# onesamblack/distributed-torch-horovod-gcp

Measured on NVIDIA H100. Metric: images/sec (whole job, device-timed, max over ranks) ResNet-50 synthetic ImageNet training, higher is better.
Workload: dtype bf16

## Files before the change

### distributed_torch_horovod_gcp_b200/csrc/conv_sm90.cu

```cuda
#include <cuda.h>
#include <cuda_bf16.h>
#include <cuda_runtime.h>
#include <limits.h>
#include <stdint.h>
#include <stdio.h>
#include <stdlib.h>
#include <string.h>

#include "sm90_common.cuh"

namespace {

constexpr int MAX_TAPS = 9;
constexpr int MAX_CLASSES = 4;

struct ConvTap {
  int amap;
  int dw, dh;
  int wcol;
};
struct ConvClass {
  int ntaps;
  int out_map;
  ConvTap taps[MAX_TAPS];
// ... 279 lines not shown
    for (int r = 0; r < R; ++r)
      for (int c = 0; c < S; ++c) {
        ConvTap& t = cl.taps[cl.ntaps++];
        t.amap = 0; t.dh = pad - r; t.dw = pad - c; t.wcol = (r * S + c) * Cin;
      }
    if (make_map4(&maps.out[0], dx, Cin, W, H, N, Cin, (uint64_t)W * Cin, (uint64_t)H * W * Cin, p.sw, p.sh, sn))
      return -1;
    maps.out[1] = maps.out[2] = maps.out[3] = maps.out[0];
  } else {
    if (make_parity_maps(maps.out, dx, Cin, W, H, N, p.sw, p.sh, sn)) return -1;
    bool any_empty = false;
    for (int ph = 0; ph < 2; ++ph)
      for (int pw = 0; pw < 2; ++pw) {
        ConvClass cl;
        memset(&cl, 0, sizeof(cl));
        cl.out_map = ph * 2 + pw;
        for (int r = 0; r < R; ++r) {
          if ((ph + pad - r) & 1) continue;
          for (int c = 0; c < S; ++c) {
            if ((pw + pad - c) & 1) continue;
            ConvTap& t = cl.taps[cl.ntaps++];
            t.amap = 0; t.dh = floordiv2(ph + pad - r); t.dw = floordiv2(pw + pad - c); t.wcol = (r * S + c) * Cin;
          }
        }
        if (cl.ntaps == 0) { any_empty = true; continue; }
        p.cls[p.num_classes++] = cl;
      }
    if (any_empty) {
      cudaError_t e = cudaMemsetAsync(dx, 0, (size_t)N * H * W * Cin * 2, st);
      if (e != cudaSuccess) return fail(cudaGetErrorString(e), (int)e);
    }
  }
  const int work = p.num_classes * p.tiles_w * p.tiles_h * p.tiles_n * p.g.num_n_blocks;
  return launch_conv<MODE_DGRAD>(maps, p, BN, work, max_ctas, st);
}

int b200dp_conv_wgrad(const void* dy, const void* x, void* dw, int N, int H, int W, int Cin, int Cout, int R, int S,
                      int stride, int pad, int splits, int block_n, int max_ctas, int accumulate, int out_bf16,
                      unsigned long long stream) {
  if (ensure_init()) return -1;
  ConvShape s{N, H, W, Cin, Cout, R, S, stride, pad, 0, 0};
  if (check_shape(s)) return -1;
  if (((uintptr_t)dy | (uintptr_t)x | (uintptr_t)dw) & 15) return fail("pointers must be 16-byte aligned");
  const int BN = pick_bn(Cin, block_n);
  if (BN < 0) return -1;
  ConvMaps maps;
  ConvParams p = conv_params();
  p.g.M = Cout; p.g.N = Cin; p.g.ldc = R * S * Cin; p.g.C = dw;
  p.g.out_mode = accumulate ? 1 : 2;
  p.g.c_bf16 = out_bf16 ? 1 : 0;
  p.g.num_m_blocks = (Cout + BLOCK_M - 1) / BLOCK_M;
  p.g.num_n_blocks = (Cin + BN - 1) / BN;
  choose_box(s.OW, s.OH, N, BLOCK_K, &p.bw, &p.bh, &p.bn);
  p.tiles_w = (s.OW + p.bw - 1) / p.bw; p.tiles_h = (s.OH + p.bh - 1) / p.bh; p.tiles_n = (N + p.bn - 1) / p.bn;
  const int kblocks = p.tiles_w * p.tiles_h * p.tiles_n;
  p.num_classes = 1;
  p.num_taps_total = R * S;
  forward_taps(p.cls[0], R, S, Cin, stride, pad);
  const int tiles = p.g.num_m_blocks * p.g.num_n_blocks * R * S;
  if (splits <= 0) {
    splits = g_num_sms / tiles;
    if (splits < 1) splits = 1;
    const int max_splits = kblocks / 8 > 1 ? kblocks / 8 : 1;
    if (splits > max_splits) splits = max_splits;
  }
  p.g.splits = normalize_splits(splits, kblocks);
// ... 20 lines not shown
```

### distributed_torch_horovod_gcp_b200/csrc/elementwise.cu

```cuda
#include <cuda_bf16.h>
#include <cuda_runtime.h>
#include <stdint.h>
#include <stdio.h>

namespace {

constexpr int THREADS = 256;

__device__ __forceinline__ void unpack8(const uint4& x, float* f) {
  const uint32_t w[4] = {x.x, x.y, x.z, x.w};
#pragma unroll
  for (int t = 0; t < 4; ++t) {
    f[2 * t] = __uint_as_float(w[t] << 16);
    f[2 * t + 1] = __uint_as_float(w[t] & 0xffff0000u);
  }
}
__device__ __forceinline__ uint4 pack8(const float* v) {
  uint32_t w[4];
#pragma unroll
  for (int t = 0; t < 4; ++t) {
    __nv_bfloat162 h = __floats2bfloat162_rn(v[2 * t], v[2 * t + 1]);
    w[t] = *reinterpret_cast<uint32_t*>(&h);
  }
  return make_uint4(w[0], w[1], w[2], w[3]);
}
__device__ __forceinline__ uint4 ldg_stream(const uint4* p) {
  uint4 v;
  asm volatile("ld.global.nc.L1::no_allocate.v4.u32 {%0,%1,%2,%3}, [%4];"
               : "=r"(v.x), "=r"(v.y), "=r"(v.z), "=r"(v.w)
               : "l"(p));
  return v;
}

constexpr int RED_MAX_BLOCKS = 256;
constexpr int RED_MAX_COLS = 2 * 2048;
__device__ float g_red_slots[RED_MAX_BLOCKS * RED_MAX_COLS];
__device__ unsigned int g_red_done;

template <int NACC, int NT>
__device__ __forceinline__ void block_reduce_to_global(float (&acc)[NACC][8], int V, float* const* outs) {
  __shared__ float sm[NT][8 + 1];
  __shared__ bool last;
  const int tid = threadIdx.x;
  const int groups = NT / V;
  const int C = V * 8;
  float* slot = g_red_slots + (size_t)blockIdx.x * (NACC * C);
#pragma unroll
  for (int q = 0; q < NACC; ++q) {
    __syncthreads();
#pragma unroll
    for (int j = 0; j < 8; ++j) sm[tid][j] = acc[q][j];
    __syncthreads();
    for (int item = tid; item < C; item += NT) {
      const int g0 = item >> 3, j = item & 7;
      float s = 0.f;
      for (int g = 0; g < groups; ++g) s += sm[g0 + g * V][j];
      slot[q * C + item] = s;
    }
  }
  __threadfence();
  __syncthreads();
  if (tid == 0) last = atomicAdd(&g_red_done, 1u) == gridDim.x - 1;
  __syncthreads();
  if (!last) return;
  __threadfence();
  for (int item = tid; item < NACC * C; item += NT) {
    float s = 0.f;
    for (unsigned b = 0; b < gridDim.x; ++b) s += __ldcg(g_red_slots + (size_t)b * (NACC * C) + item);
    outs[item / C][item % C] += s;
  }
  if (tid == 0) g_red_done = 0u;
}

constexpr int RTHREADS = 1024;

__device__ __forceinline__ uint4 ld_or_zero(const uint4* p, long long i, long long n) {
  return i < n ? ldg_stream(p + i) : make_uint4(0, 0, 0, 0);
}

__global__ void __launch_bounds__(RTHREADS, 1) bn_stats_kernel(const uint4* __restrict__ x, float* sum,
                                                               float* sumsq, long long nvec, int V) {
  constexpr int U = 8;
  float acc[2][8];
#pragma unroll
  for (int j = 0; j < 8; ++j) acc[0][j] = acc[1][j] = 0.f;
  const long long stride = (long long)gridDim.x * RTHREADS;
  for (long long i = (long long)blockIdx.x * RTHREADS + threadIdx.x; i < nvec; i += U * stride) {
    uint4 raw[U];
#pragma unroll
    for (int u = 0; u < U; ++u) raw[u] = ld_or_zero(x, i + u * stride, nvec);
#pragma unroll
    for (int u = 0; u < U; ++u) {
      float f[8];
      unpack8(raw[u], f);
#pragma unroll
      for (int j = 0; j < 8; ++j) {
        acc[0][j] += f[j];
        acc[1][j] = fmaf(f[j], f[j], acc[1][j]);
      }
    }
  }
  float* outs[2] = {sum, sumsq};
  block_reduce_to_global<2, RTHREADS>(acc, V, outs);
}

__device__ __forceinline__ float ld_param(const void* p, int c, int bf16) {
  return bf16 ? __bfloat162float(reinterpret_cast<const __nv_bfloat16*>(p)[c])
              : reinterpret_cast<const float*>(p)[c];
}
__device__ __forceinline__ void st_param(void* p, int c, int bf16, float v) {
  if (bf16) reinterpret_cast<__nv_bfloat16*>(p)[c] = __float2bfloat16_rn(v);
  else reinterpret_cast<float*>(p)[c] = v;
}

__global__ void bn_finalize_kernel(float* sum, float* sumsq, const void* gamma,
                                   const void* beta, float* mean, float* invstd, float* a, float* b,
                                   void* running_mean, void* running_var, float count, float eps,
                                   float momentum, int C, int pbf16, int rezero = 0,
                                   long long* num_batches_tracked = nullptr) {
  const int c = blockIdx.x * blockDim.x + threadIdx.x;
  if (c == 0 && num_batches_tracked != nullptr) *num_batches_tracked += 1;
  if (c >= C) return;
  const float m = sum[c] / count;
  const float var = fmaxf(sumsq[c] / count - m * m, 0.f);
  if (rezero) {
    sum[c] = 0.f;
    sumsq[c] = 0.f;
  }
  const float is = rsqrtf(var + eps);
  mean[c] = m;
  invstd[c] = is;
  const float g = gamma ? ld_param(gamma, c, pbf16) : 1.f;
  a[c] = g * is;
  b[c] = (beta ? ld_param(beta, c, pbf16) : 0.f) - m * g * is;
  if (running_mean) {
    const float unbiased = var * (count / fmaxf(count - 1.f, 1.f));
    st_param(running_mean, c, pbf16, (1.f - momentum) * ld_param(running_mean, c, pbf16) + momentum * m);
    st_param(running_var, c, pbf16,
             (1.f - momentum) * ld_param(running_var, c, pbf16) + momentum * unbiased);
  }
}

__global__ void __launch_bounds__(THREADS, 4) bn_apply_kernel(const uint4* __restrict__ x,
                                                              const uint4* __restrict__ res, uint4* y,
                                                              const float* __restrict__ a,
                                                              const float* __restrict__ b, long long nvec,
                                                              int V, int relu, uint8_t* __restrict__ mask) {
  constexpr int U = 4;
  const long long stride = (long long)gridDim.x * THREADS;
  const long long i0 = (long long)blockIdx.x * THREADS + threadIdx.x;
  if (i0 >= nvec) return;
  const int cg = (int)(i0 % V);
  float av[8], bv[8];
#pragma unroll
  for (int j = 0; j < 8; ++j) {
    av[j] = a[cg * 8 + j];
    bv[j] = b[cg * 8 + j];
  }
  for (long long i = i0; i < nvec; i += U * stride) {
    uint4 rx[U], rr[U];
#pragma unroll
    for (int u = 0; u < U; ++u) rx[u] = ld_or_zero(x, i + u * stride, nvec);
    if (res) {
#pragma unroll
      for (int u = 0; u < U; ++u) rr[u] = ld_or_zero(res, i + u * stride, nvec);
    }
#pragma unroll
    for (int u = 0; u < U; ++u) {
      if (i + u * stride >= nvec) break;
      float f[8];
      unpack8(rx[u], f);
#pragma unroll
      for (int j = 0; j < 8; ++j) f[j] = fmaf(f[j], av[j], bv[j]);
      if (res) {
        float r[8];
        unpack8(rr[u], r);
#pragma unroll
        for (int j = 0; j < 8; ++j) f[j] += r[j];
      }
      if (relu) {
        if (mask) {
          uint32_t m = 0;
#pragma unroll
          for (int j = 0; j < 8; ++j) m |= (f[j] > 0.f ? 1u : 0u) << j;
          mask[i + u * stride] = (uint8_t)m;
        }
#pragma unroll
        for (int j = 0; j < 8; ++j) f[j] = fmaxf(f[j], 0.f);
      }
      y[i + u * stride] = pack8(f);
    }
  }
}

__global__ void __launch_bounds__(RTHREADS, 1) bn_bwd_reduce_kernel(
    const uint4* __restrict__ dy, const uint4* __restrict__ x, const uint8_t* __restrict__ mask,
    const float* __restrict__ mean, float* sum_dy, float* sum_dy_xc, long long nvec, int V, int relu) {
  constexpr int U = 2;
  float acc[2][8];
#pragma unroll
  for (int j = 0; j < 8; ++j) acc[0][j] = acc[1][j] = 0.f;
  const long long stride = (long long)gridDim.x * RTHREADS;
  const long long i0 = (long long)blockIdx.x * RTHREADS + threadIdx.x;
  float mv[8];
  {
    const int cg = (int)(i0 % V);
#pragma unroll
    for (int j = 0; j < 8; ++j) mv[j] = mean[cg * 8 + j];
  }
  for (long long i = i0; i < nvec; i += U * stride) {
    uint4 rg[U], rx[U];
    uint32_t rm[U];
#pragma unroll
    for (int u = 0; u < U; ++u) {
      rg[u] = ld_or_zero(dy, i + u * stride, nvec);
      rx[u] = ld_or_zero(x, i + u * stride, nvec);
      rm[u] = (relu && i + u * stride < nvec) ? (uint32_t)__ldg(mask + i + u * stride) : 0xffu;
    }
#pragma unroll
    for (int u = 0; u < U; ++u) {
      float g[8], xv[8];
      unpack8(rg[u], g);
      unpack8(rx[u], xv);
#pragma unroll
      for (int j = 0; j < 8; ++j) g[j] = ((rm[u] >> j) & 1u) ? g[j] : 0.f;
#pragma unroll
      for (int j = 0; j < 8; ++j) {
        acc[0][j] += g[j];
        acc[1][j] = fmaf(g[j], xv[j] - mv[j], acc[1][j]);
      }
    }
  }
  float* outs[2] = {sum_dy, sum_dy_xc};
  block_reduce_to_global<2, RTHREADS>(acc, V, outs);
}

__global__ void __launch_bounds__(THREADS, 4) bn_bwd_apply_kernel(
    const uint4* __restrict__ dy, const uint4* __restrict__ x, const uint8_t* __restrict__ mask, uint4* dx,
    uint4* dres, const float* __restrict__ mean, const float* __restrict__ invstd,
    const float* __restrict__ scale_a, const float* __restrict__ sum_dy,
    const float* __restrict__ sum_dy_xhat, float inv_count, long long nvec, int V, int relu,
    void* dgamma, void* dbeta, int pbf16) {
  constexpr int U = 2;
  const long long stride = (long long)gridDim.x * THREADS;
  const long long i0 = (long long)blockIdx.x * THREADS + threadIdx.x;
  if (blockIdx.x == 0 && dgamma != nullptr) {
    for (int c = threadIdx.x; c < V * 8; c += THREADS) {
      st_param(dbeta, c, pbf16, sum_dy[c]);
      st_param(dgamma, c, pbf16, sum_dy_xhat[c] * invstd[c]);
    }
  }
  if (i0 >= nvec) return;
  const int cg = (int)(i0 % V);
  float mv[8], iv[8], k1[8], k2[8], sc[8];
#pragma unroll
  for (int j = 0; j < 8; ++j) {
    const int c = cg * 8 + j;
    mv[j] = mean[c];
    iv[j] = invstd[c];
    sc[j] = scale_a[c];
    k1[j] = sum_dy[c] * inv_count;
    k2[j] = sum_dy_xhat[c] * iv[j] * inv_count;
  }
  for (long long i = i0; i < nvec; i += U * stride) {
    uint4 rg[U], rx[U];
    uint32_t rm[U];
#pragma unroll
    for (int u = 0; u < U; ++u) {
      rg[u] = ld_or_zero(dy, i + u * stride, nvec);
      rx[u] = ld_or_zero(x, i + u * stride, nvec);
      rm[u] = (relu && i + u * stride < nvec) ? (uint32_t)__ldg(mask + i + u * stride) : 0xffu;
    }
#pragma unroll
    for (int u = 0; u < U; ++u) {
      if (i + u * stride >= nvec) break;
      float g[8], xv[8], o[8];
      unpack8(rg[u], g);
      unpack8(rx[u], xv);
#pragma unroll
      for (int j = 0; j < 8; ++j) g[j] = ((rm[u] >> j) & 1u) ? g[j] : 0.f;
#pragma unroll
      for (int j = 0; j < 8; ++j) {
        const float xhat = (xv[j] - mv[j]) * iv[j];
        o[j] = sc[j] * (g[j] - k1[j] - xhat * k2[j]);
      }
      dx[i + u * stride] = pack8(o);
      if (dres) dres[i + u * stride] = pack8(g);
    }
  }
}

constexpr int LN_WARPS = 16;

template <int VPL>
__global__ void __launch_bounds__(LN_WARPS * 32) ln_fwd_kernel(const uint4* __restrict__ x, uint4* __restrict__ y,
                                                               const void* gamma, const void* beta,
                                                               float* __restrict__ mean, float* __restrict__ rstd,
// ... 357 lines not shown
  if (blocks < 1) blocks = 1;
  return (int)blocks;
}

template <bool OUT_BF16>
__global__ void cast_acc_zero_kernel(float* __restrict__ src, void* __restrict__ dst, long long n4,
                                     int accumulate, int zero_src) {
  const long long stride = (long long)gridDim.x * blockDim.x;
  for (long long i = (long long)blockIdx.x * blockDim.x + threadIdx.x; i < n4; i += stride) {
    float4 v = reinterpret_cast<float4*>(src)[i];
    if (zero_src) reinterpret_cast<float4*>(src)[i] = make_float4(0.f, 0.f, 0.f, 0.f);
    if (OUT_BF16) {
      uint2* d = reinterpret_cast<uint2*>(dst) + i;
      if (accumulate) {
        const uint2 o = *d;
        v.x += __uint_as_float(o.x << 16); v.y += __uint_as_float(o.x & 0xffff0000u);
        v.z += __uint_as_float(o.y << 16); v.w += __uint_as_float(o.y & 0xffff0000u);
      }
      __nv_bfloat162 lo = __floats2bfloat162_rn(v.x, v.y), hi = __floats2bfloat162_rn(v.z, v.w);
      *d = make_uint2(*reinterpret_cast<uint32_t*>(&lo), *reinterpret_cast<uint32_t*>(&hi));
    } else {
      float4* d = reinterpret_cast<float4*>(dst) + i;
      if (accumulate) { const float4 o = *d; v.x += o.x; v.y += o.y; v.z += o.z; v.w += o.w; }
      *d = v;
    }
  }
}

bool shape_ok(int C) {
  const int V = C / 8;
  return C % 8 == 0 && V >= 1 && V <= THREADS && (THREADS % V) == 0;
}

}

extern "C" {

const char* b200dp_ew_last_error() { return g_err; }

int b200dp_cast_acc_zero(void* src, void* dst, long long n, int out_bf16, int accumulate, int zero_src,
                         unsigned long long stream) {
  if (n % 4) {
    snprintf(g_err, sizeof(g_err), "cast_acc_zero: n must be a multiple of 4");
    return -1;
  }
  const long long n4 = n / 4;
  int grid = (int)((n4 + 255) / 256);
  if (grid > reduce_grid() * 8) grid = reduce_grid() * 8;
  if (grid < 1) grid = 1;
  cudaStream_t st = (cudaStream_t)(uintptr_t)stream;
  if (out_bf16) cast_acc_zero_kernel<true><<<grid, 256, 0, st>>>((float*)src, dst, n4, accumulate, zero_src);
  else cast_acc_zero_kernel<false><<<grid, 256, 0, st>>>((float*)src, dst, n4, accumulate, zero_src);
  cudaError_t e = cudaGetLastError();
  if (e != cudaSuccess) return fail("cast_acc_zero launch", e);
  return 0;
}

int b200dp_bn_supported(int C) { return shape_ok(C) ? 1 : 0; }

int b200dp_bn_fwd(const void* x, const void* res, void* y, const void* gamma, const void* beta,
                  float* stats, float* mean, float* invstd, float* a, float* b, void* running_mean,
                  void* running_var, long long M, int C, float eps, float momentum, int relu,
                  int param_bf16, int have_stats, void* relu_mask, void* num_batches_tracked,
                  unsigned long long stream) {
  if (!shape_ok(C)) {
    snprintf(g_err, sizeof(g_err), "unsupported channel count %d", C);
    return -1;
  }
  cudaStream_t st = (cudaStream_t)(uintptr_t)stream;
  const int V = C / 8;
  const long long nvec = M * V;
  cudaError_t e = cudaSuccess;
  const int grid = grid_for(nvec, V);
  if (!have_stats) {
    e = cudaMemsetAsync(stats, 0, sizeof(float) * 2 * C, st);
    if (e != cudaSuccess) return fail("memset", e);
    bn_stats_kernel<<<reduce_grid(), RTHREADS, 0, st>>>((const uint4*)x, stats, stats + C, nvec, V);
  }
  bn_finalize_kernel<<<(C + 127) / 128, 128, 0, st>>>(stats, stats + C, gamma, beta, mean, invstd, a, b,
                                                      running_mean, running_var, (float)M, eps, momentum, C,
                                                      param_bf16, have_stats == 2 ? 1 : 0,
                                                      (long long*)num_batches_tracked);
  bn_apply_kernel<<<grid, THREADS, 0, st>>>((const uint4*)x, (const uint4*)res, (uint4*)y, a, b, nvec, V,
                                            relu, (uint8_t*)relu_mask);
  e = cudaGetLastError();
  if (e != cudaSuccess) return fail("bn_fwd launch", e);
  return 0;
}

int b200dp_bn_stats(const void* x, float* stats, long long M, int C, unsigned long long stream) {
  if (!shape_ok(C)) return -1;
  cudaStream_t st = (cudaStream_t)(uintptr_t)stream;
  cudaError_t e = cudaMemsetAsync(stats, 0, sizeof(float) * 2 * C, st);
  if (e != cudaSuccess) return fail("memset", e);
  bn_stats_kernel<<<reduce_grid(), RTHREADS, 0, st>>>((const uint4*)x, stats, stats + C, (long long)M * (C / 8),
                                                      C / 8);
  e = cudaGetLastError();
  if (e != cudaSuccess) return fail("bn_stats launch", e);
  return 0;
}

int b200dp_bn_fwd_sync(const void* x, const void* res, void* y, const void* gamma, const void* beta,
                       const float* stats, float* mean, float* invstd, float* a, float* b, void* running_mean,
                       void* running_var, long long M_local, double count, int C, float eps, float momentum,
                       int relu, int param_bf16, void* relu_mask, unsigned long long stream) {
  if (!shape_ok(C)) return -1;
  cudaStream_t st = (cudaStream_t)(uintptr_t)stream;
  const int V = C / 8;
  const long long nvec = M_local * V;
  bn_finalize_kernel<<<(C + 127) / 128, 128, 0, st>>>(const_cast<float*>(stats), const_cast<float*>(stats) + C, gamma,
                                                      beta, mean, invstd, a, b, running_mean, running_var,
                                                      (float)count, eps, momentum, C, param_bf16);
  bn_apply_kernel<<<grid_for(nvec, V), THREADS, 0, st>>>((const uint4*)x, (const uint4*)res, (uint4*)y, a, b, nvec,
                                                         V, relu, (uint8_t*)relu_mask);
  cudaError_t e = cudaGetLastError();
  if (e != cudaSuccess) return fail("bn_fwd_sync launch", e);
  return 0;
}

int b200dp_bn_bwd_reduce(const void* dy, const void* x, const void* relu_mask, const float* mean, float* sums,
                         long long M, int C, int relu, unsigned long long stream) {
  if (!shape_ok(C)) return -1;
  cudaStream_t st = (cudaStream_t)(uintptr_t)stream;
  cudaError_t e = cudaMemsetAsync(sums, 0, sizeof(float) * 2 * C, st);
  if (e != cudaSuccess) return fail("memset", e);
  bn_bwd_reduce_kernel<<<reduce_grid(), RTHREADS, 0, st>>>((const uint4*)dy, (const uint4*)x,
                                                           (const uint8_t*)relu_mask, mean, sums, sums + C,
                                                           (long long)M * (C / 8), C / 8, relu);
  e = cudaGetLastError();
  if (e != cudaSuccess) return fail("bn_bwd_reduce launch", e);
  return 0;
}

int b200dp_bn_bwd_apply(const void* dy, const void* x, const void* relu_mask, void* dx, void* dres,
                        const float* scale_a, const float* mean, const float* invstd, const float* sums,
                        double count, long long M, int C, int relu, unsigned long long stream) {
  if (!shape_ok(C)) return -1;
  const int V = C / 8;
  const long long nvec = M * V;
  bn_bwd_apply_kernel<<<grid_for(nvec, V), THREADS, 0, (cudaStream_t)(uintptr_t)stream>>>(
      (const uint4*)dy, (const uint4*)x, (const uint8_t*)relu_mask, (uint4*)dx, (uint4*)dres, mean, invstd, scale_a,
      sums, sums + C, (float)(1.0 / count), nvec, V, relu, nullptr, nullptr, 0);
  cudaError_t e = cudaGetLastError();
  if (e != cudaSuccess) return fail("bn_bwd_apply launch", e);
  return 0;
}

int b200dp_bn_apply(const void* x, const void* res, void* y, const float* a, const float* b, long long M,
                    int C, int relu, unsigned long long stream) {
  if (!shape_ok(C)) return -1;
  const int V = C / 8;
  const long long nvec = M * V;
  bn_apply_kernel<<<grid_for(nvec, V), THREADS, 0, (cudaStream_t)(uintptr_t)stream>>>(
      (const uint4*)x, (const uint4*)res, (uint4*)y, a, b, nvec, V, relu, nullptr);
  cudaError_t e = cudaGetLastError();
  if (e != cudaSuccess) return fail("bn_apply launch", e);
  return 0;
}

int b200dp_bn_bwd(const void* dy, const void* x, const void* relu_mask, void* dx, void* dres, const float* scale_a,
                  const float* mean, const float* invstd, float* sums, void* dgamma, void* dbeta,
                  int param_bf16, long long M, int C, int relu, unsigned long long stream) {
  if (!shape_ok(C)) return -1;
  cudaStream_t st = (cudaStream_t)(uintptr_t)stream;
  const int V = C / 8;
  const long long nvec = M * V;
  cudaError_t e = cudaMemsetAsync(sums, 0, sizeof(float) * 2 * C, st);
  if (e != cudaSuccess) return fail("memset", e);
  const int grid = grid_for(nvec, V);
  bn_bwd_reduce_kernel<<<reduce_grid(), RTHREADS, 0, st>>>((const uint4*)dy, (const uint4*)x,
                                                           (const uint8_t*)relu_mask, mean, sums, sums + C,
                                                           nvec, V, relu);
  bn_bwd_apply_kernel<<<grid, THREADS, 0, st>>>((const uint4*)dy, (const uint4*)x, (const uint8_t*)relu_mask,
                                                (uint4*)dx, (uint4*)dres, mean, invstd, scale_a, sums,
                                                sums + C, 1.0f / (float)M, nvec, V, relu, dgamma, dbeta,
                                                param_bf16);
  e = cudaGetLastError();
  if (e != cudaSuccess) return fail("bn_bwd launch", e);
  return 0;
}

int b200dp_maxpool_fwd(const void* x, void* y, void* idx, int N, int H, int W, int C,
                       unsigned long long stream) {
  if (C % 8) return -1;
  const int OH = (H + 2 - 3) / 2 + 1, OW = (W + 2 - 3) / 2 + 1, V = C / 8;
  const long long total = (long long)N * OH * OW * V;
  int grid = (int)((total + THREADS - 1) / THREADS);
  if (grid > reduce_grid() * 16) grid = reduce_grid() * 16;
  maxpool_fwd_kernel<<<grid, THREADS, 0, (cudaStream_t)(uintptr_t)stream>>>((const uint4*)x, (uint4*)y,
                                                                             (uint2*)idx, N, H, W, OH, OW, V);
  cudaError_t e = cudaGetLastError();
  if (e != cudaSuccess) return fail("maxpool_fwd launch", e);
  return 0;
}

int b200dp_maxpool_bwd(const void* dy, const void* idx, void* dx, int N, int H, int W, int C,
                       unsigned long long stream) {
  if (C % 8) return -1;
  const int OH = (H + 2 - 3) / 2 + 1, OW = (W + 2 - 3) / 2 + 1, V = C / 8;
  if (H % 2 == 0 && W % 2 == 0) {
    const long long patches = (long long)N * (H / 2) * (W / 2) * V;
    int pgrid = (int)((patches + THREADS - 1) / THREADS);
    if (pgrid > reduce_grid() * 16) pgrid = reduce_grid() * 16;
    maxpool_bwd_patch_kernel<<<pgrid, THREADS, 0, (cudaStream_t)(uintptr_t)stream>>>(
        (const uint4*)dy, (const uint2*)idx, (uint4*)dx, N, H, W, OH, OW, V);
    cudaError_t pe = cudaGetLastError();
    if (pe != cudaSuccess) return fail("maxpool_bwd launch", pe);
    return 0;
  }
  const long long total = (long long)N * H * W * V;
// ... 93 lines not shown
```

### distributed_torch_horovod_gcp_b200/csrc/gemm_sm90.cu

```cuda
#include <cuda.h>
#include <cuda_bf16.h>
#include <cuda_runtime.h>
#include <stdint.h>

#include "sm90_common.cuh"

namespace {

template <int BN, bool A_MN, bool B_MN>
struct GemmWork {
  static constexpr bool kStats = true, kSplitK = true;
  const CUtensorMap *a, *b, *c;
  const GemmParams& p;
  int tiles, items, kb_per_split;

  __device__ GemmWork(const CUtensorMap* a_, const CUtensorMap* b_, const CUtensorMap* c_, const GemmParams& p_)
      : a(a_), b(b_), c(c_), p(p_), tiles(p_.num_m_blocks * p_.num_n_blocks), items(tiles * p_.splits),
        kb_per_split((p_.num_k_blocks + p_.splits - 1) / p_.splits) {}
  __device__ void prefetch() const {
    tma_prefetch_desc(a);
    tma_prefetch_desc(b);
    if (p.out_mode == 0) tma_prefetch_desc(c);
  }
  __device__ int m_idx(int tile) const {
// ... 65 lines not shown
}

extern "C" {

const char* b200dp_gemm_last_error() { return g_err; }

int b200dp_gemm_bf16(const void* A, const void* B, void* C, int M, int N, int K, int lda, int ldb, int ldc,
                     int a_mn, int b_mn, const void* bias_bf16, const void* bias_f32, const void* residual,
                     void* preact, int act, int out_mode, int out_bf16, float alpha, int splits, int block_n,
                     int max_ctas, float* stats, const void* res_mask, unsigned long long stream) {
  if (ensure_init()) return -1;
  if (M <= 0 || N <= 0 || K <= 0) return fail("bad shape");
  if ((N % 8) || (lda % 8) || (ldb % 8) || (ldc % 4) || ((out_mode == 0 || out_bf16) && (ldc % 8)))
    return fail("alignment: N, lda, ldb, ldc must be multiples of 8");
  if (((uintptr_t)A | (uintptr_t)B | (uintptr_t)C) & 15) return fail("pointers must be 16-byte aligned");
  const int BN = pick_bn(N, block_n);
  if (BN < 0) return -1;
  GemmParams p{};
  p.M = M; p.N = N; p.ldc = ldc;
  p.num_m_blocks = (M + BLOCK_M - 1) / BLOCK_M;
  p.num_n_blocks = (N + BN - 1) / BN;
  p.num_k_blocks = (K + BLOCK_K - 1) / BLOCK_K;
  p.splits = normalize_splits(splits, p.num_k_blocks);
  if (p.splits > 1 && (out_mode == 0 || bias_bf16 || bias_f32 || residual || preact || act))
    return fail("split-K requires out_mode 1/2 without bias, residual or activation");
  p.act = act; p.out_mode = out_mode; p.c_bf16 = out_bf16 ? 1 : 0; p.C = C; p.bias = bias_bf16; p.bias_f32 = bias_f32;
  p.residual = residual; p.preact = preact; p.alpha = alpha;
  p.stats = stats;
  p.res_mask = reinterpret_cast<const unsigned char*>(res_mask);
  if (res_mask != nullptr && (residual == nullptr || preact != nullptr || act > 2 || out_mode != 0 || (N % 64) ||
                              ldc != N))
    return fail("res_mask: plain bf16 residual, dense rows and N % 64 == 0 required");
  if (stats != nullptr && (N > STATS_MAX_N || out_mode != 0)) return fail("stats: N <= 2048 and bf16 output required");
  p.n_fastest = ((size_t)N * (size_t)K * 2 <= ((size_t)20 << 20)) ? 1 : 0;
  CUtensorMap ma, mb, mc;
  if (a_mn ? make_map2(&ma, A, K, M, lda, BLOCK_K) : make_map2(&ma, A, M, K, lda, BLOCK_M)) return -1;
  if (b_mn ? make_map2(&mb, B, K, N, ldb, BLOCK_K) : make_map2(&mb, B, N, K, ldb, BN)) return -1;
  if (out_mode == 0) {
    if (make_map2(&mc, C, M, N, ldc, 32)) return -1;
  } else {
    mc = ma;
  }
  cudaStream_t st = (cudaStream_t)(uintptr_t)stream;
  if (p.splits > 1) p.splitk_slice = (long long)M * ldc;
  return run_splitk(p, p.num_m_blocks * p.num_n_blocks, st,
                    [&] { return launch_bn(BN, a_mn, b_mn, ma, mb, mc, p, max_ctas, st); });
}

}
```

### distributed_torch_horovod_gcp_b200/csrc/sm90_common.cuh

```cuda
#pragma once
#include <cuda.h>
#include <cuda_bf16.h>
#include <cuda_runtime.h>
#include <stdint.h>
#include <stdio.h>

namespace {

constexpr int BLOCK_M = 128;
constexpr int BLOCK_K = 64;
constexpr int WGMMA_K = 16;
constexpr int NUM_THREADS = 384;
constexpr int SMEM_LIMIT = 232448;

struct GemmParams {
  int M, N;
  int ldc;
  int num_m_blocks, num_n_blocks, num_k_blocks;
  int splits;
  int act;
  int out_mode;
  int c_bf16;
  void* C;
  const void* bias;
  const void* bias_f32;
  const void* residual;
  void* preact;
  int n_fastest;
  float alpha;
  const unsigned char* res_mask;
  float* stats;
  float* splitk_ws;
  int* splitk_count;
  long long splitk_slice;
};

constexpr int STATS_MAX_N = 2048;
constexpr int STATS_WARP_FLOATS = 256;
constexpr int STATS_SMEM_BYTES = 8 * STATS_WARP_FLOATS * 4;

__device__ __forceinline__ uint32_t smem_u32(const void* p) {
  return static_cast<uint32_t>(__cvta_generic_to_shared(p));
}
__device__ __forceinline__ void mbar_init(uint64_t* bar, uint32_t count) {
  asm volatile("mbarrier.init.shared::cta.b64 [%0], %1;" ::"r"(smem_u32(bar)), "r"(count));
}
__device__ __forceinline__ void mbar_expect_tx(uint64_t* bar, uint32_t bytes) {
  asm volatile("mbarrier.arrive.expect_tx.shared::cta.b64 _, [%0], %1;" ::"r"(smem_u32(bar)),
               "r"(bytes)
               : "memory");
}
__device__ __forceinline__ void mbar_arrive(uint64_t* bar) {
  asm volatile("mbarrier.arrive.shared::cta.b64 _, [%0];" ::"r"(smem_u32(bar)) : "memory");
}
__device__ __forceinline__ void mbar_wait(uint64_t* bar, uint32_t parity) {
  uint32_t done = 0;
  unsigned long long t0 = 0;
  for (uint32_t tries = 0; !done; ++tries) {
    asm volatile(
        "{\n\t"
        ".reg .pred p;\n\t"
        "mbarrier.try_wait.parity.shared::cta.b64 p, [%1], %2;\n\t"
        "selp.u32 %0, 1, 0, p;\n\t"
        "}\n"
        : "=r"(done)
        : "r"(smem_u32(bar)), "r"(parity)
        : "memory");
// ... 562 lines not shown
  uint8_t* smem_store = smem + C::STAGES * C::STAGE_BYTES;
  uint64_t* bars = reinterpret_cast<uint64_t*>(smem_store + C::STORE_BYTES);
  uint64_t* full_bar = bars;
  uint64_t* empty_bar = bars + C::STAGES;
  float* s_stats = reinterpret_cast<float*>(reinterpret_cast<uint8_t*>(bars) + 256);
  const bool want_stats = Work::kStats && p.stats != nullptr && p.out_mode == 0;
  if (want_stats) stats_zero(s_stats, NUM_THREADS, p.N);

  const int warp = threadIdx.x >> 5;
  const int lane = threadIdx.x & 31;

  if (warp == 0 && lane == 0) {
    wk.prefetch();
    for (int i = 0; i < C::STAGES; ++i) {
      mbar_init(&full_bar[i], 1);
      mbar_init(&empty_bar[i], 2);
    }
    asm volatile("fence.mbarrier_init.release.cluster;" ::: "memory");
  }
  __syncthreads();

  if (warp < 4) {
    asm volatile("setmaxnreg.dec.sync.aligned.u32 40;" ::: "memory");
    if (warp == 0 && elect_one()) {
      int stage = 0;
      uint32_t phase = 0;
      auto next = [&]() {
        mbar_wait(&empty_bar[stage], phase ^ 1);
        mbar_expect_tx(&full_bar[stage], C::STAGE_BYTES);
        const Stage s{smem_a + stage * C::A_BYTES, smem_b + stage * C::B_BYTES, &full_bar[stage]};
        if (++stage == C::STAGES) { stage = 0; phase ^= 1; }
        return s;
      };
      for (int w = blockIdx.x; w < wk.items; w += gridDim.x) wk.load(w, next);
    }
  } else {
    asm volatile("setmaxnreg.inc.sync.aligned.u32 232;" ::: "memory");
    const int cw = warp - 4;
    const int wg = cw >> 2;
    const int r0 = wg * 64 + (cw & 3) * 16;
    const int q = cw & 3;
    const int half = cw >> 2;
    const int c_begin = (BN >= 128) ? half * (BN / 2) : 0;
    const int c_end = (BN >= 128) ? c_begin + BN / 2 : (half == 0 ? BN : 0);
    const int epi_tid = cw * 32 + lane;
    float* my_stats = s_stats + cw * STATS_WARP_FLOATS;
    const uint32_t stg = smem_u32(smem_store);
    __shared__ int s_last;
    int stats_n = -1;
    int stage = 0;
    uint32_t phase = 0;
    float d[BN / 2];
    for (int w = blockIdx.x; w < wk.items; w += gridDim.x) {
      const Slab s = wk.slab(w, q);
      wg_mainloop<BN, A_MN, B_MN, C::STAGES, C::A_BYTES, C::B_BYTES>(d, smem_u32(smem_a), smem_u32(smem_b), full_bar,
                                                                     empty_bar, stage, phase, wk.num_kb(w), wg);
      if (want_stats && s.n_idx != stats_n) {
        if (stats_n >= 0) stats_flush<BN>(p, s_stats, stats_n, epi_tid);
        stats_n = s.n_idx;
      }
      const bool res = p.residual != nullptr && p.out_mode != 1;
      uint4 rv[BN / 16];
      if (res) res_load<BN>(p, rv, s.m_idx, r0, s.n_idx, lane);
      if (p.out_mode == 0) {
        if (lane == 0) tma_store_wait_read<0>();
        named_bar(1, 256);
      }
      if (res) {
        __syncwarp();
        res_stage<BN>(rv, stg, r0, lane);
        __syncwarp();
      }
      epilogue_frag<BN>(p, d, stg, wg, s.m_idx, s.n_idx, s.split, s.c_off);
      if (p.out_mode == 0) {
        fence_async_smem();
        named_bar(1, 256);
        store_slab<BN>(p, s.map_c, smem_store, q, lane, s.m_row0, s.n_idx, c_begin, c_end, s.at,
                       want_stats ? my_stats : nullptr);
      }
      if (Work::kSplitK && p.splits > 1) splitk_finish_tile(p, s.tile, s.m_idx, s.n_idx, BN, s.c_off, epi_tid, &s_last);
    }
    if (want_stats && stats_n >= 0) stats_flush<BN>(p, s_stats, stats_n, epi_tid);
    if (want_stats) stats_finalize(p, epi_tid);
    if (p.out_mode == 0 && lane == 0) tma_store_wait_all();
  }
}
// ... 72 lines not shown
  cudaError_t e = cudaGetLastError();
  if (e != cudaSuccess) return fail(cudaGetErrorString(e), (int)e);
  return 0;
}

template <class Launch>
int run_splitk(GemmParams& p, int tiles, cudaStream_t st, Launch&& launch) {
  void* ws = nullptr;
  if (p.splits > 1) {
    const size_t slices = (size_t)p.splits * (size_t)p.splitk_slice * sizeof(float);
    cudaError_t e = cudaMallocAsync(&ws, slices + (size_t)tiles * sizeof(int), st);
    if (e == cudaSuccess) {
      p.splitk_ws = reinterpret_cast<float*>(ws);
      p.splitk_count = reinterpret_cast<int*>(reinterpret_cast<char*>(ws) + slices);
      e = cudaMemsetAsync(p.splitk_count, 0, (size_t)tiles * sizeof(int), st);
    }
    if (e != cudaSuccess) return fail(cudaGetErrorString(e), (int)e);
  }
  const int rc = launch();
  if (ws != nullptr) {
    cudaError_t e = cudaFreeAsync(ws, st);
    if (e != cudaSuccess && rc == 0) return fail(cudaGetErrorString(e), (int)e);
  }
  return rc;
}

int normalize_splits(int splits, int kblocks) {
  if (splits > kblocks) splits = kblocks;
  if (splits < 1) splits = 1;
  const int per = (kblocks + splits - 1) / splits;
  return (kblocks + per - 1) / per;
}

int pick_bn(int n, int block_n) {
  if (block_n == 0) return n > 64 ? 128 : 64;
  if (block_n == 256) return 128;
  if (block_n != 64 && block_n != 128) return fail("block_n must be 64/128/256");
  return block_n;
}

}
```

### distributed_torch_horovod_gcp_b200/ops/bottleneck.py

```python
from __future__ import annotations

import torch

from . import bn as _bn
from . import conv as _conv
from . import gemm as _gemm
from . import grad_sink


def _units(block):
    ds = [(block.downsample[0], block.downsample[1])] if block.downsample is not None else []
    return [(block.conv1, block.bn1), (block.conv2, block.bn2)] + ds + [(block.conv3, block.bn3)]


def supported(x: torch.Tensor, block) -> bool:
    if _bn._lib is None or not _bn._nhwc_ok(x):
        return False
    for conv, bn in _units(block):
        if not (bn.training and bn.weight is not None and _bn._lib.b200dp_bn_supported(conv.out_channels)):
            return False
        if not _bn._is_gemm_conv(x, conv) and (conv in (block.conv1, block.conv3) or conv.bias is not None or
                                               not _conv.supported(x, conv.weight, conv.stride, conv.padding,
                                                                   conv.dilation, conv.groups)):
            return False
# ... 17 lines not shown
                       N * H * W, C, x.shape[1], stats=stats).view(N, H, W, C).permute(0, 3, 1, 2)
    else:
        w = _conv._krsc(conv.weight)
        y = _conv.conv_fprop(x, w, conv.stride[0], conv.padding[0], stats)
    out, mask, ws = _bn.bn_forward(y, bn, residual, relu, stats, need[1:])
    return out, (x, w, y, mask, *ws)


class _BottleneckFn(torch.autograd.Function):

    @staticmethod
    def forward(ctx, block, x, *params):
        units = _units(block)
        need = [ctx.needs_input_grad[2 + 3 * i:5 + 3 * i] for i in range(len(units))]
        h, s1 = _unit_forward(x, *units[0], True, None, need[0])
        h, s2 = _unit_forward(h, *units[1], True, None, need[1])
        identity, sd = _unit_forward(x, *units[2], False, None, need[2]) if len(units) == 4 else (x, ())
        y, s3 = _unit_forward(h, *units[-1], True, identity, need[-1])
        ctx.save_for_backward(*s1, *s2, *sd, *s3)
        ctx.block = block
        return y

    @staticmethod
    def backward(ctx, dy):
        units, need = _units(ctx.block), ctx.needs_input_grad
        n = len(units)
        saved = [ctx.saved_tensors[7 * i:7 * i + 7] for i in range(n)]
        grads = [None] * n

        def unit(i, dout, mask, want_dx, residual=None, res_mask=None):
            (conv, bn), (x, w, y, _, *ws), need_dw = units[i], saved[i], need[2 + 3 * i]
            dz, dgamma, dbeta, _ = _bn.bn_backward(dout, bn, y, mask, ws)
            dx = dw = None
            if w.dim() == 2:
                N, C, H, W = x.shape
                if want_dx:
                    dx = _gemm.dgrad(_rows(dz), w, residual, res_mask).view(N, H, W, C).permute(0, 3, 1, 2)
                if need_dw:
                    dw = _gemm.wgrad(_rows(dz), _rows(x), w.shape[0], C, N * H * W, w.dtype, owner=conv.weight)
                    dw = dw.view(conv.weight.shape) if dw is not None else None
            else:
                if want_dx:
                    dx = _conv.conv_dgrad(dz, w, x.shape, conv.stride[0], conv.padding[0])
                if need_dw:
                    dw = _conv.conv_wgrad(dz, x, conv.weight, conv.stride[0], conv.padding[0])
            grads[i] = (dw, dgamma, dbeta)
            return dx

        dy, mask3 = _bn._cl(dy), saved[-1][3]
        d = unit(1, unit(n - 1, dy, mask3, True), saved[1][3], True)
        skip, skip_mask = (unit(2, dy, mask3, need[1]), None) if n == 4 else (dy, mask3)
        dx = unit(0, d, saved[0][3], need[1], _rows(skip) if need[1] else None, skip_mask)
        return (None, dx) + tuple(g for unit_grads in grads for g in unit_grads)


def bottleneck(x: torch.Tensor, block) -> torch.Tensor:
    params = [p for conv, bn in _units(block) for p in (conv.weight, bn.weight, bn.bias)]
    return _BottleneckFn.apply(block, x, *params)
```

### distributed_torch_horovod_gcp_b200/ops/grad_sink.py

```python
from __future__ import annotations

import os
from typing import Callable, Optional, Tuple

import torch

_ENABLED = os.environ.get("B200DP_GRAD_SINK", "1") == "1"


class ParamSink:
    __slots__ = ("uses", "multi", "manual", "passes_done", "_fire")

    def __init__(self, passes_done: Callable[[], int], fire: Callable[[], None]):
        self.uses = 0
        self.multi = False
        self.manual = False
        self.passes_done = passes_done
        self._fire = fire

    def fire(self):
        self._fire()
        self.manual = True

    def reset(self):
        self.uses = 0
        self.multi = False

    def reset_step(self):
        self.reset()
        self.manual = False


def note_forward(weight) -> None:
    sink = getattr(weight, "_b200dp_sink", None)
    if sink is not None:
        sink.uses += 1
        if sink.uses > 1:
            sink.multi = True


def begin(weight, krsc: bool = False) -> Tuple[Optional[torch.Tensor], bool, Optional[Callable[[], None]]]:
    sink = getattr(weight, "_b200dp_sink", None)
    if not _ENABLED or sink is None or sink.multi or sink.uses != 1:
        return None, False, None
    g = weight.grad
    if g is None or g.dtype != weight.dtype or g.data_ptr() % 16:
        return None, False, None
    if krsc:
        if g.dim() != 4 or not g.is_contiguous(memory_format=torch.channels_last):
            return None, False, None
    elif not g.is_contiguous():
        if not (g.dim() == 4 and g.shape[2] == 1 and g.shape[3] == 1 and
                g.is_contiguous(memory_format=torch.channels_last)):
            return None, False, None
    return g, sink.passes_done() > 0, sink.fire


class GradBox:

    def __init__(self, *args, **kwargs):
        raise RuntimeError("GradBox was removed: a ResNet bottleneck block runs as one autograd node "
                           "(ops/bottleneck.py) that adds the skip gradient in conv1's dgrad itself")
```

### distributed_torch_horovod_gcp_b200/ops/kernels.py

```python
from __future__ import annotations

import os
from typing import Dict

import torch

_HAVE: Dict[str, bool] = {}
_LIB = None
_TRIED = False


def _load():
    global _LIB, _TRIED
    if _TRIED:
        return _LIB
    _TRIED = True
    from ..runtime import lib as rtlib
    _LIB = rtlib.load_kernels()
    if _LIB is not None:
        from . import _bind
        _bind.register(_LIB, _HAVE)
    return _LIB


def enabled_for(x: torch.Tensor) -> bool:
    if not x.is_cuda or os.environ.get("B200DP_DISABLE_KERNELS", "0") == "1":
        return False
    if _load() is None:
        return False
    return torch.cuda.get_device_capability(x.device)[0] == 9


def has(op: str) -> bool:
    _load()
    return _HAVE.get(op, False)


def __getattr__(name):
    from . import _bind
    if hasattr(_bind, name):
        return getattr(_bind, name)
    raise AttributeError(name)
```

Measured before the change: 5705.

## Reverse walk order in BN apply and GEMM/conv kernels for L2 handoff

Adds an L2 handoff mode, enabled by default through an env flag. In it, BN apply and BN backward apply kernels and order-free GEMM and conv dgrad kernels walk their tiles in reverse, so each consumer starts on the data its producer wrote last, which is likely still in L2. It also drops the memset before the BN backward reduce by having the final reduction block store instead of accumulate. It reorders wgrad before dgrad and defers grad-sink fire callbacks until both finish. The risks are extra index arithmetic, and the reorder only pays off when tensors partly fit in the H100's L2.

```diff
diff --git a/distributed_torch_horovod_gcp_b200/csrc/conv_sm90.cu b/distributed_torch_horovod_gcp_b200/csrc/conv_sm90.cu
--- a/distributed_torch_horovod_gcp_b200/csrc/conv_sm90.cu
+++ b/distributed_torch_horovod_gcp_b200/csrc/conv_sm90.cu
@@ -335,6 +335,7 @@
     }
   }
   const int work = p.num_classes * p.tiles_w * p.tiles_h * p.tiles_n * p.g.num_n_blocks;
+  walk_order(p.g, true);
   return launch_conv<MODE_DGRAD>(maps, p, BN, work, max_ctas, st);
 }
 
diff --git a/distributed_torch_horovod_gcp_b200/csrc/elementwise.cu b/distributed_torch_horovod_gcp_b200/csrc/elementwise.cu
--- a/distributed_torch_horovod_gcp_b200/csrc/elementwise.cu
+++ b/distributed_torch_horovod_gcp_b200/csrc/elementwise.cu
@@ -2,6 +2,7 @@
 #include <cuda_runtime.h>
 #include <stdint.h>
 #include <stdio.h>
+#include <stdlib.h>
 
 namespace {
 
@@ -37,8 +38,15 @@
 __device__ float g_red_slots[RED_MAX_BLOCKS * RED_MAX_COLS];
 __device__ unsigned int g_red_done;
 
+__device__ __forceinline__ float zero_plus(float v) {
+  float o;
+  asm("add.rn.f32 %0, %1, %2;" : "=f"(o) : "f"(0.0f), "f"(v));
+  return o;
+}
+
 template <int NACC, int NT>
-__device__ __forceinline__ void block_reduce_to_global(float (&acc)[NACC][8], int V, float* const* outs) {
+__device__ __forceinline__ void block_reduce_to_global(float (&acc)[NACC][8], int V, float* const* outs,
+                                                       bool store = false) {
   __shared__ float sm[NT][8 + 1];
   __shared__ bool last;
   const int tid = threadIdx.x;
@@ -67,7 +75,8 @@
   for (int item = tid; item < NACC * C; item += NT) {
     float s = 0.f;
     for (unsigned b = 0; b < gridDim.x; ++b) s += __ldcg(g_red_slots + (size_t)b * (NACC * C) + item);
-    outs[item / C][item % C] += s;
+    float& o = outs[item / C][item % C];
+    o = store ? zero_plus(s) : o + s;
   }
   if (tid == 0) g_red_done = 0u;
 }
@@ -76,6 +85,10 @@
 
 __device__ __forceinline__ uint4 ld_or_zero(const uint4* p, long long i, long long n) {
   return i < n ? ldg_stream(p + i) : make_uint4(0, 0, 0, 0);
+}
+
+__device__ __forceinline__ long long walk_top(long long i0, long long chunk, long long nvec) {
+  return i0 + (nvec - 1 - i0) / chunk * chunk;
 }
 
 __global__ void __launch_bounds__(RTHREADS, 1) bn_stats_kernel(const uint4* __restrict__ x, float* sum,
@@ -141,6 +154,7 @@
   }
 }
 
+template <bool REVERSE>
 __global__ void __launch_bounds__(THREADS, 4) bn_apply_kernel(const uint4* __restrict__ x,
                                                               const uint4* __restrict__ res, uint4* y,
                                                               const float* __restrict__ a,
@@ -157,7 +171,8 @@
     av[j] = a[cg * 8 + j];
     bv[j] = b[cg * 8 + j];
   }
-  for (long long i = i0; i < nvec; i += U * stride) {
+  for (long long i = REVERSE ? walk_top(i0, U * stride, nvec) : i0; (unsigned long long)i < (unsigned long long)nvec;
+       i += REVERSE ? -U * stride : U * stride) {
     uint4 rx[U], rr[U];
 #pragma unroll
     for (int u = 0; u < U; ++u) rx[u] = ld_or_zero(x, i + u * stride, nvec);
@@ -195,7 +210,7 @@
 
 __global__ void __launch_bounds__(RTHREADS, 1) bn_bwd_reduce_kernel(
     const uint4* __restrict__ dy, const uint4* __restrict__ x, const uint8_t* __restrict__ mask,
-    const float* __restrict__ mean, float* sum_dy, float* sum_dy_xc, long long nvec, int V, int relu) {
+    const float* __restrict__ mean, float* sum_dy, float* sum_dy_xc, long long nvec, int V, int relu, int store) {
   constexpr int U = 2;
   float acc[2][8];
 #pragma unroll
@@ -232,9 +247,10 @@
     }
   }
   float* outs[2] = {sum_dy, sum_dy_xc};
-  block_reduce_to_global<2, RTHREADS>(acc, V, outs);
-}
-
+  block_reduce_to_global<2, RTHREADS>(acc, V, outs, store != 0);
+}
+
+template <bool REVERSE>
 __global__ void __launch_bounds__(THREADS, 4) bn_bwd_apply_kernel(
     const uint4* __restrict__ dy, const uint4* __restrict__ x, const uint8_t* __restrict__ mask, uint4* dx,
     uint4* dres, const float* __restrict__ mean, const float* __restrict__ invstd,
@@ -262,7 +278,8 @@
     k1[j] = sum_dy[c] * inv_count;
     k2[j] = sum_dy_xhat[c] * iv[j] * inv_count;
   }
-  for (long long i = i0; i < nvec; i += U * stride) {
+  for (long long i = REVERSE ? walk_top(i0, U * stride, nvec) : i0; (unsigned long long)i < (unsigned long long)nvec;
+       i += REVERSE ? -U * stride : U * stride) {
     uint4 rg[U], rx[U];
     uint32_t rm[U];
 #pragma unroll
@@ -686,11 +703,25 @@
   return C % 8 == 0 && V >= 1 && V <= THREADS && (THREADS % V) == 0;
 }
 
+int g_l2_handoff = -1;
+
+auto bn_apply(bool reverse) { return reverse ? bn_apply_kernel<true> : bn_apply_kernel<false>; }
+auto bn_bwd_apply(bool reverse) { return reverse ? bn_bwd_apply_kernel<true> : bn_bwd_apply_kernel<false>; }
+
 }
 
 extern "C" {
 
 const char* b200dp_ew_last_error() { return g_err; }
+
+int b200dp_l2_handoff() {
+  if (g_l2_handoff < 0) {
+    const char* e = getenv("B200DP_L2_HANDOFF");
+    g_l2_handoff = (e != nullptr && e[0] == '0') ? 0 : 1;
+  }
+  return g_l2_handoff;
+}
+void b200dp_set_l2_handoff(int on) { g_l2_handoff = on ? 1 : 0; }
 
 int b200dp_cast_acc_zero(void* src, void* dst, long long n, int out_bf16, int accumulate, int zero_src,
                          unsigned long long stream) {
@@ -735,8 +766,8 @@
                                                       running_mean, running_var, (float)M, eps, momentum, C,
                                                       param_bf16, have_stats == 2 ? 1 : 0,
                                                       (long long*)num_batches_tracked);
-  bn_apply_kernel<<<grid, THREADS, 0, st>>>((const uint4*)x, (const uint4*)res, (uint4*)y, a, b, nvec, V,
-                                            relu, (uint8_t*)relu_mask);
+  bn_apply(b200dp_l2_handoff())<<<grid, THREADS, 0, st>>>((const uint4*)x, (const uint4*)res, (uint4*)y, a, b, nvec,
+                                                          V, relu, (uint8_t*)relu_mask);
   e = cudaGetLastError();
   if (e != cudaSuccess) return fail("bn_fwd launch", e);
   return 0;
@@ -765,8 +796,8 @@
   bn_finalize_kernel<<<(C + 127) / 128, 128, 0, st>>>(const_cast<float*>(stats), const_cast<float*>(stats) + C, gamma,
                                                       beta, mean, invstd, a, b, running_mean, running_var,
                                                       (float)count, eps, momentum, C, param_bf16);
-  bn_apply_kernel<<<grid_for(nvec, V), THREADS, 0, st>>>((const uint4*)x, (const uint4*)res, (uint4*)y, a, b, nvec,
-                                                         V, relu, (uint8_t*)relu_mask);
+  bn_apply_kernel<false><<<grid_for(nvec, V), THREADS, 0, st>>>((const uint4*)x, (const uint4*)res, (uint4*)y, a, b,
+                                                                nvec, V, relu, (uint8_t*)relu_mask);
   cudaError_t e = cudaGetLastError();
   if (e != cudaSuccess) return fail("bn_fwd_sync launch", e);
   return 0;
@@ -780,7 +811,7 @@
   if (e != cudaSuccess) return fail("memset", e);
   bn_bwd_reduce_kernel<<<reduce_grid(), RTHREADS, 0, st>>>((const uint4*)dy, (const uint4*)x,
                                                            (const uint8_t*)relu_mask, mean, sums, sums + C,
-                                                           (long long)M * (C / 8), C / 8, relu);
+                                                           (long long)M * (C / 8), C / 8, relu, 0);
   e = cudaGetLastError();
   if (e != cudaSuccess) return fail("bn_bwd_reduce launch", e);
   return 0;
@@ -792,7 +823,7 @@
   if (!shape_ok(C)) return -1;
   const int V = C / 8;
   const long long nvec = M * V;
-  bn_bwd_apply_kernel<<<grid_for(nvec, V), THREADS, 0, (cudaStream_t)(uintptr_t)stream>>>(
+  bn_bwd_apply_kernel<false><<<grid_for(nvec, V), THREADS, 0, (cudaStream_t)(uintptr_t)stream>>>(
       (const uint4*)dy, (const uint4*)x, (const uint8_t*)relu_mask, (uint4*)dx, (uint4*)dres, mean, invstd, scale_a,
       sums, sums + C, (float)(1.0 / count), nvec, V, relu, nullptr, nullptr, 0);
   cudaError_t e = cudaGetLastError();
@@ -805,7 +836,7 @@
   if (!shape_ok(C)) return -1;
   const int V = C / 8;
   const long long nvec = M * V;
-  bn_apply_kernel<<<grid_for(nvec, V), THREADS, 0, (cudaStream_t)(uintptr_t)stream>>>(
+  bn_apply_kernel<false><<<grid_for(nvec, V), THREADS, 0, (cudaStream_t)(uintptr_t)stream>>>(
       (const uint4*)x, (const uint4*)res, (uint4*)y, a, b, nvec, V, relu, nullptr);
   cudaError_t e = cudaGetLastError();
   if (e != cudaSuccess) return fail("bn_apply launch", e);
@@ -819,17 +850,14 @@
   cudaStream_t st = (cudaStream_t)(uintptr_t)stream;
   const int V = C / 8;
   const long long nvec = M * V;
-  cudaError_t e = cudaMemsetAsync(sums, 0, sizeof(float) * 2 * C, st);
-  if (e != cudaSuccess) return fail("memset", e);
   const int grid = grid_for(nvec, V);
   bn_bwd_reduce_kernel<<<reduce_grid(), RTHREADS, 0, st>>>((const uint4*)dy, (const uint4*)x,
                                                            (const uint8_t*)relu_mask, mean, sums, sums + C,
-                                                           nvec, V, relu);
-  bn_bwd_apply_kernel<<<grid, THREADS, 0, st>>>((const uint4*)dy, (const uint4*)x, (const uint8_t*)relu_mask,
-                                                (uint4*)dx, (uint4*)dres, mean, invstd, scale_a, sums,
-                                                sums + C, 1.0f / (float)M, nvec, V, relu, dgamma, dbeta,
-                                                param_bf16);
-  e = cudaGetLastError();
+                                                           nvec, V, relu, 1);
+  bn_bwd_apply(b200dp_l2_handoff())<<<grid, THREADS, 0, st>>>(
+      (const uint4*)dy, (const uint4*)x, (const uint8_t*)relu_mask, (uint4*)dx, (uint4*)dres, mean, invstd, scale_a,
+      sums, sums + C, 1.0f / (float)M, nvec, V, relu, dgamma, dbeta, param_bf16);
+  cudaError_t e = cudaGetLastError();
   if (e != cudaSuccess) return fail("bn_bwd launch", e);
   return 0;
 }
diff --git a/distributed_torch_horovod_gcp_b200/csrc/gemm_sm90.cu b/distributed_torch_horovod_gcp_b200/csrc/gemm_sm90.cu
--- a/distributed_torch_horovod_gcp_b200/csrc/gemm_sm90.cu
+++ b/distributed_torch_horovod_gcp_b200/csrc/gemm_sm90.cu
@@ -121,6 +121,7 @@
                               ldc != N))
     return fail("res_mask: plain bf16 residual, dense rows and N % 64 == 0 required");
   if (stats != nullptr && (N > STATS_MAX_N || out_mode != 0)) return fail("stats: N <= 2048 and bf16 output required");
+  walk_order(p, !a_mn && b_mn);
   p.n_fastest = ((size_t)N * (size_t)K * 2 <= ((size_t)20 << 20)) ? 1 : 0;
   CUtensorMap ma, mb, mc;
   if (a_mn ? make_map2(&ma, A, K, M, lda, BLOCK_K) : make_map2(&ma, A, M, K, lda, BLOCK_M)) return -1;
diff --git a/distributed_torch_horovod_gcp_b200/csrc/sm90_common.cuh b/distributed_torch_horovod_gcp_b200/csrc/sm90_common.cuh
--- a/distributed_torch_horovod_gcp_b200/csrc/sm90_common.cuh
+++ b/distributed_torch_horovod_gcp_b200/csrc/sm90_common.cuh
@@ -4,6 +4,8 @@
 #include <cuda_runtime.h>
 #include <stdint.h>
 #include <stdio.h>
+
+extern "C" int b200dp_l2_handoff();
 
 namespace {
 
@@ -33,6 +35,7 @@
   float* splitk_ws;
   int* splitk_count;
   long long splitk_slice;
+  int reverse;
 };
 
 constexpr int STATS_MAX_N = 2048;
@@ -661,7 +664,7 @@
         if (++stage == C::STAGES) { stage = 0; phase ^= 1; }
         return s;
       };
-      for (int w = blockIdx.x; w < wk.items; w += gridDim.x) wk.load(w, next);
+      for (int w = blockIdx.x; w < wk.items; w += gridDim.x) wk.load(p.reverse ? wk.items - 1 - w : w, next);
     }
   } else {
     asm volatile("setmaxnreg.inc.sync.aligned.u32 232;" ::: "memory");
@@ -680,7 +683,8 @@
     int stage = 0;
     uint32_t phase = 0;
     float d[BN / 2];
-    for (int w = blockIdx.x; w < wk.items; w += gridDim.x) {
+    for (int pos = blockIdx.x; pos < wk.items; pos += gridDim.x) {
+      const int w = p.reverse ? wk.items - 1 - pos : pos;
       const Slab s = wk.slab(w, q);
       wg_mainloop<BN, A_MN, B_MN, C::STAGES, C::A_BYTES, C::B_BYTES>(d, smem_u32(smem_a), smem_u32(smem_b), full_bar,
                                                                      empty_bar, stage, phase, wk.num_kb(w), wg);
@@ -819,6 +823,10 @@
   return (kblocks + per - 1) / per;
 }
 
+void walk_order(GemmParams& p, bool order_free) {
+  p.reverse = (order_free && p.stats == nullptr && b200dp_l2_handoff()) ? 1 : 0;
+}
+
 int pick_bn(int n, int block_n) {
   if (block_n == 0) return n > 64 ? 128 : 64;
   if (block_n == 256) return 128;
diff --git a/distributed_torch_horovod_gcp_b200/ops/bottleneck.py b/distributed_torch_horovod_gcp_b200/ops/bottleneck.py
--- a/distributed_torch_horovod_gcp_b200/ops/bottleneck.py
+++ b/distributed_torch_horovod_gcp_b200/ops/bottleneck.py
@@ -73,18 +73,19 @@
             (conv, bn), (x, w, y, _, *ws), need_dw = units[i], saved[i], need[2 + 3 * i]
             dz, dgamma, dbeta, _ = _bn.bn_backward(dout, bn, y, mask, ws)
             dx = dw = None
-            if w.dim() == 2:
-                N, C, H, W = x.shape
-                if want_dx:
-                    dx = _gemm.dgrad(_rows(dz), w, residual, res_mask).view(N, H, W, C).permute(0, 3, 1, 2)
-                if need_dw:
-                    dw = _gemm.wgrad(_rows(dz), _rows(x), w.shape[0], C, N * H * W, w.dtype, owner=conv.weight)
-                    dw = dw.view(conv.weight.shape) if dw is not None else None
-            else:
-                if want_dx:
-                    dx = _conv.conv_dgrad(dz, w, x.shape, conv.stride[0], conv.padding[0])
-                if need_dw:
-                    dw = _conv.conv_wgrad(dz, x, conv.weight, conv.stride[0], conv.padding[0])
+            with grad_sink.held():
+                if w.dim() == 2:
+                    N, C, H, W = x.shape
+                    if need_dw:
+                        dw = _gemm.wgrad(_rows(dz), _rows(x), w.shape[0], C, N * H * W, w.dtype, owner=conv.weight)
+                        dw = dw.view(conv.weight.shape) if dw is not None else None
+                    if want_dx:
+                        dx = _gemm.dgrad(_rows(dz), w, residual, res_mask).view(N, H, W, C).permute(0, 3, 1, 2)
+                else:
+                    if need_dw:
+                        dw = _conv.conv_wgrad(dz, x, conv.weight, conv.stride[0], conv.padding[0])
+                    if want_dx:
+                        dx = _conv.conv_dgrad(dz, w, x.shape, conv.stride[0], conv.padding[0])
             grads[i] = (dw, dgamma, dbeta)
             return dx
 
diff --git a/distributed_torch_horovod_gcp_b200/ops/grad_sink.py b/distributed_torch_horovod_gcp_b200/ops/grad_sink.py
--- a/distributed_torch_horovod_gcp_b200/ops/grad_sink.py
+++ b/distributed_torch_horovod_gcp_b200/ops/grad_sink.py
@@ -1,11 +1,13 @@
 from __future__ import annotations
 
+import contextlib
 import os
-from typing import Callable, Optional, Tuple
+from typing import Callable, List, Optional, Tuple
 
 import torch
 
 _ENABLED = os.environ.get("B200DP_GRAD_SINK", "1") == "1"
+_held: Optional[List[Callable[[], None]]] = None
 
 
 class ParamSink:
@@ -53,7 +55,23 @@
         if not (g.dim() == 4 and g.shape[2] == 1 and g.shape[3] == 1 and
                 g.is_contiguous(memory_format=torch.channels_last)):
             return None, False, None
+    if _held is not None:
+        queue = _held
+        return g, sink.passes_done() > 0, lambda: queue.append(sink.fire)
     return g, sink.passes_done() > 0, sink.fire
+
+
+@contextlib.contextmanager
+def held():
+    global _held
+    prev, _held = _held, []
+    try:
+        yield
+        pending = _held
+    finally:
+        _held = prev
+    for fire in pending:
+        fire()
 
 
 class GradBox:
diff --git a/distributed_torch_horovod_gcp_b200/ops/kernels.py b/distributed_torch_horovod_gcp_b200/ops/kernels.py
--- a/distributed_torch_horovod_gcp_b200/ops/kernels.py
+++ b/distributed_torch_horovod_gcp_b200/ops/kernels.py
@@ -36,6 +36,22 @@
     return _HAVE.get(op, False)
 
 
+def set_l2_handoff(on: bool) -> bool:
+    lib = _load()
+    if lib is None:
+        raise RuntimeError("libb200dp_kernels.so not loaded")
+    prev = bool(lib.b200dp_l2_handoff())
+    lib.b200dp_set_l2_handoff(int(bool(on)))
+    return prev
+
+
+def l2_handoff() -> bool:
+    lib = _load()
+    if lib is None:
+        raise RuntimeError("libb200dp_kernels.so not loaded")
+    return bool(lib.b200dp_l2_handoff())
+
+
 def __getattr__(name):
     from . import _bind
     if hasattr(_bind, name):
```

Result: faster. 5800, median of 6 (+1.7%).
